# zhangganlin/vista-slam

Hardware: AMD Instinct MI355X
Metric: STA image-pairs/sec @512x384 (higher is better)
Workload: dtype f16x3-split MFMA (3 fp16 products) in the transformer and the pose head; fp16 MFMA + one block-scaled fp8 correction MFMA in the DPT head's convolutions; fp32 accumulate; 1 GPU; 512x384 batch=8 pairs/GPU STA two-view forward (BASELINE configs[1]); pairs_per_gpu=8, H=384, W=512, precision=f16x3h, parallelism=single GPU

## Files before the change

include/sta_mi355_debug.h:

```cpp
#ifndef STA_MI355_DEBUG_H
#define STA_MI355_DEBUG_H
#include "sta_mi355.h"
#ifdef __cplusplus
extern "C" {
#endif

STA_API int sta_set_gemm_variant(sta_handle* h, int variant);

STA_API int sta_debug_pick_family(int amode, int epi, long long M, int N, int K, int split, int cstride, int Ho, int Wo);

STA_API int sta_debug_gemm_plan(int amode, int epi, int M_all, int N, int K, int precision, int mx, int tail_hint, int forced_variant, int* out);

STA_API int sta_debug_last_gemm_plan(sta_handle* h, int* out);

STA_API int sta_debug_qkv_pair_plan(int precision, int M, int N_a, int N_b, int K, int mx_a, int mx_b, int tail_hint, int forced_variant, int* out);

STA_API int sta_debug_qkv_pair(sta_handle* h, const float* x_a, const float* w_a, const float* bias_a, const float* x_b,
                       const float* w_b, const float* bias_b, int S, int ntok, int K, int C, int wp,
                       float* q_a, float* k_a, float* vt_a, float* k_b, float* vt_b, void* stream);

STA_API int sta_debug_gemm(sta_handle* h, const float* A, const float* W, const float* bias, int M, int N, int K,
                   int act, int via_f16, const float* resid, float* out, void* stream);

STA_API int sta_debug_qkv_rope(sta_handle* h, const float* x, const float* W, const float* bias, int S, int ntok, int K, int C,
// ... 14 lines not shown

STA_API int sta_debug_convt(sta_handle* h, const float* x, const float* w, const float* bias, int n, int H, int W, int C, int k,
                    float* out, void* stream);

STA_API int sta_debug_up2(sta_handle* h, const float* x, int n, int H, int W, int C, int Hc, int Wc, float* out, void* stream);

STA_API int sta_debug_layernorm(sta_handle* h, const float* x, const float* g, const float* b, int M, int C, float eps,
                        float* out32, float* out_planes, void* stream);

STA_API int sta_debug_head_final(sta_handle* h, const float* x, const float* w, const float* bias, int64_t npix,
                         float* pts, float* conf, void* stream);

STA_API int sta_debug_svd_orthogonalize(sta_handle* h, const float* m, float* r, int B, void* stream);

STA_API int sta_kernel_timing_dump(sta_handle* h, int cap, double* flops, float* ms, int* variant, int* n_out);

STA_API int sta_kernel_stamps_dump(sta_handle* h, int cap, double* out6, int* n_out);

STA_API int sta_bench_gemm_stamps(sta_handle* h, int M, int N, int K, int resid, double* out, unsigned long long* raw_host, int raw_cap, void* stream);

STA_API int sta_bench_gemm(sta_handle* h, int M, int N, int K, int iters, int tile, int ablation, float* ms_out, void* stream);
STA_API float sta_bench_gemm_last_ghz(void);
STA_API int sta_bench_attention(sta_handle* h, int S, int heads, int nq, int nk, int pose, int iters, int which, float* ms_out, void* stream);

#ifdef __cplusplus
}
#endif
#endif
```

vista_slam_amd/_lib.py:

```python
import ctypes as C
import os

PKG = os.path.dirname(os.path.abspath(__file__))
LIB_PATH = os.path.join(PKG, "libsta_mi355.so")
TEST_LIB_PATH = os.path.join(PKG, "libsta_mi355_test.so")

STA_PREC_F16 = 1
STA_PREC_F16X3 = 3
STA_PREC_F16X3H = 5
STA_PREC_F16X3M = 6
PRECISIONS = {"f16": STA_PREC_F16, "f16x3": STA_PREC_F16X3, "f16x3h": STA_PREC_F16X3H, "f16x3m": STA_PREC_F16X3M}


class StaConfig(C.Structure):
    _fields_ = [("patch_size", C.c_int32), ("enc_embed_dim", C.c_int32), ("enc_depth", C.c_int32),
                ("enc_num_heads", C.c_int32), ("dec_embed_dim", C.c_int32), ("dec_depth", C.c_int32),
                ("dec_num_heads", C.c_int32), ("mlp_ratio", C.c_int32), ("rope_base", C.c_float),
                ("ln_eps", C.c_float), ("precision", C.c_int32)]


_vp, _i, _i64, _f = C.c_void_p, C.c_int, C.c_int64, C.c_float
_fp = C.c_void_p

SIGNATURES = {
# ... 38 lines not shown
    "sta_flops_per_pair": (C.c_double, [_vp, _i, _i]),
    "sta_workspace_bytes": (_i64, [_vp]),
    "sta_weight_bytes": (_i64, [_vp]),
    "sta_enable_stage_timing": (_i, [_vp, _i]),
    "sta_get_stage_ms": (_i, [_vp, C.POINTER(_f)]),
    "sta_kernel_timing": (_i, [_vp, _i]),
    "sta_kernel_timing_read": (_i, [_vp, _i, C.POINTER(_i), C.POINTER(C.c_double), C.POINTER(C.c_double), C.POINTER(C.c_double)]),
    "sta_kernel_clock_read": (_i, [_vp, C.POINTER(C.c_float)]),
    "sta_kernel_timing_filter": (_i, [_vp, _i, _i, _i, _i, _i]),
    "sta_kernel_timing_dump_shapes": (_i, [_vp, _i, C.POINTER(_i), C.POINTER(C.c_float), C.POINTER(_i), C.POINTER(_i)]),
    "sta_range_report": (_i, [_vp, C.POINTER(C.c_ulonglong), _i]),
    "sta_last_error": (C.c_char_p, []),
    "sta_version": (C.c_char_p, []),
}

TEST_SIGNATURES = {
    "sta_set_gemm_variant": (_i, [_vp, _i]),
    "sta_kernel_timing_dump": (_i, [_vp, _i, C.POINTER(C.c_double), C.POINTER(C.c_float), C.POINTER(_i), C.POINTER(_i)]),
    "sta_kernel_stamps_dump": (_i, [_vp, _i, C.POINTER(C.c_double), C.POINTER(_i)]),
    "sta_bench_gemm_stamps": (_i, [_vp, _i, _i, _i, _i, C.POINTER(C.c_double), C.POINTER(C.c_ulonglong), _i, _vp]),
    "sta_bench_gemm": (_i, [_vp, _i, _i, _i, _i, _i, _i, C.POINTER(_f), _vp]),
    "sta_bench_gemm_last_ghz": (C.c_float, []),
    "sta_bench_attention": (_i, [_vp, _i, _i, _i, _i, _i, _i, _i, C.POINTER(_f), _vp]),
    "sta_debug_gemm": (_i, [_vp, _fp, _fp, _fp, _i, _i, _i, _i, _i, _fp, _fp, _vp]),
    "sta_debug_qkv_rope": (_i, [_vp, _fp, _fp, _fp, _i, _i, _i, _i, _i, _i, _fp, _fp, _fp, _vp]),
    "sta_debug_attention": (_i, [_vp, _fp, _fp, _fp, _i, _i, _i, _i, _i, _fp, _vp]),
    "sta_debug_attention_pose": (_i, [_vp, _fp, _fp, _fp, _i, _i, _i, _i, _fp, _vp]),
    "sta_debug_set_tail_hint": (_i, [_vp, _i]),
    "sta_debug_set_option": (_i, [_vp, _i, _i]),
    "sta_debug_pick_family": (_i, [_i, _i, C.c_longlong, _i, _i, _i, _i, _i, _i]),
    "sta_debug_gemm_plan": (_i, [_i, _i, _i, _i, _i, _i, _i, _i, _i, C.POINTER(_i)]),
    "sta_debug_last_gemm_plan": (_i, [_vp, C.POINTER(_i)]),
    "sta_debug_qkv_pair_plan": (_i, [_i, _i, _i, _i, _i, _i, _i, _i, _i, C.POINTER(_i)]),
    "sta_debug_qkv_pair": (_i, [_vp, _fp, _fp, _fp, _fp, _fp, _fp, _i, _i, _i, _i, _i, _fp, _fp, _fp, _fp, _fp, _vp]),
    "sta_debug_conv3x3": (_i, [_vp, _fp, _fp, _fp, _i, _i, _i, _i, _i, _i, _i, _i, _fp, _fp, _vp]),
    "sta_debug_convt": (_i, [_vp, _fp, _fp, _fp, _i, _i, _i, _i, _i, _fp, _vp]),
    "sta_debug_up2": (_i, [_vp, _fp, _i, _i, _i, _i, _i, _i, _fp, _vp]),
    "sta_debug_layernorm": (_i, [_vp, _fp, _fp, _fp, _i, _i, _f, _fp, _fp, _vp]),
    "sta_debug_head_final": (_i, [_vp, _fp, _fp, _fp, _i64, _fp, _fp, _vp]),
    "sta_debug_svd_orthogonalize": (_i, [_vp, _fp, _fp, _i, _vp]),
}

_lib = None
_test_lib = None


# ... 73 lines not shown
```

vista_slam_amd/csrc/attention.h:

```cpp
#pragma once
#include "sta_common.h"
#include <type_traits>

__device__ __forceinline__ void glds16(const void* gsrc, void* lds_dst_wave_base);

struct AttnParams {
    const f16* Q_hi; const f16* Q_lo; const f16* K_hi; const f16* K_lo; const f16* Vt_hi; const f16* Vt_lo;
    f16* O_hi; f16* O_lo; int ldo;
    int S, heads, nq, nk, npad;
    int kv_shift;
    float scale_log2e;
    unsigned long long* range;
    int prefetch;
    int pose;
};

#define ATT_KV 64
#define ATT_TILE_BYTES (64 * 128)

template <bool SPLIT>
constexpr int attn_smem_bytes(int stages = 2) { return stages * (SPLIT ? 4 : 2) * ATT_TILE_BYTES; }
#define ATT_PREFETCH_TILES 4

template <bool SPLIT>
__device__ __forceinline__ void attn_pose_query(const AttnParams& p, char* smem) {
    const int tid = threadIdx.x, lane = tid & 63, wave = tid >> 6;
    const int sh = blockIdx.x;
    const int s = sh / p.heads, h = sh - s * p.heads;
    const int skv = (s + p.kv_shift) % p.S;
    const size_t qoff = ((size_t)(s * p.heads + h) * p.npad + p.nq) * 64;
    const size_t koff = (size_t)(skv * p.heads + h) * p.npad * 64;
    const size_t voff = (size_t)(skv * p.heads + h) * 64 * p.npad;
    float* pl = reinterpret_cast<float*>(smem);
    float* red = pl + p.npad;
    float q[64];
#pragma unroll
    for (int c = 0; c < 8; ++c) {
// ... 42 lines not shown
        H8 a[2], b[2];
#pragma unroll
        for (int u = 0; u < 2; ++u) { a[u].u = ldg16(vh + c0 + u * 8); if (SPLIT) b[u].u = ldg16(vl + c0 + u * 8); }
#pragma unroll
        for (int u = 0; u < 2; ++u) {
            const int c = c0 + u * 8;
            const float4 p0 = *reinterpret_cast<const float4*>(pl + c), p1 = *reinterpret_cast<const float4*>(pl + c + 4);
            const float pe[8] = {p0.x, p0.y, p0.z, p0.w, p1.x, p1.y, p1.z, p1.w};
#pragma unroll
            for (int e = 0; e < 8; ++e) o = __builtin_fmaf(pe[e], (float)a[u].e[e] + (SPLIT ? (float)b[u].e[e] : 0.f), o);
        }
    }
    red[8 + wave * 64 + lane] = o;
    __syncthreads();
    if (wave != 0) return;
    o = (red[8 + lane] + red[8 + 64 + lane]) + (red[8 + 128 + lane] + red[8 + 192 + lane]);
    o /= (red[4] + red[5]) + (red[6] + red[7]);
    const int64_t orow = (int64_t)p.S * p.nq + s, orows = (int64_t)p.S * p.nq + p.S;
    const size_t oo = blk_off<SPLIT>(orow, h * 64 + lane, orows);
    if (SPLIT) { f16 hh, ll; split_f16(o, hh, ll, p.range); p.O_hi[oo] = hh; p.O_hi[oo + 32] = ll; }
    else p.O_hi[oo] = to_f16_sat(o, p.range);
}

template <bool SPLIT>
__global__ __launch_bounds__(256, 2) void attn_kernel(const AttnParams p) {
    extern __shared__ __attribute__((aligned(16))) char smem[];
    constexpr int NPL = SPLIT ? 2 : 1;
    constexpr int STAGE = 2 * NPL * ATT_TILE_BYTES;
    const int npose_blocks = p.pose == 1 ? p.S * p.heads : 0;
    const int nqe = p.nq + (p.pose == 2 ? 1 : 0);
    if ((int)blockIdx.x < npose_blocks) { attn_pose_query<SPLIT>(p, smem); return; }
    const int tid = threadIdx.x, lane = tid & 63;
    const int wave = __builtin_amdgcn_readfirstlane(tid >> 6);
    const int l31 = lane & 31, lhi = lane >> 5;
    const int nqb = (nqe + 127) / 128;
    const int nwg = nqb * p.heads * p.S;
    int logical;
    {
        const int bid = blockIdx.x - npose_blocks, q = nwg / 8, r = nwg % 8, xcd = bid % 8;
        logical = (xcd < r ? xcd * (q + 1) : r * (q + 1) + (xcd - r) * q) + bid / 8;
    }
    const int qb = logical % nqb;
    const int h = (logical / nqb) % p.heads, s = logical / (nqb * p.heads);
    const int skv = (s + p.kv_shift) % p.S;
    const int q0 = qb * 128 + wave * 32;

    const size_t qoff = (size_t)(s * p.heads + h) * p.npad * 64;
    const size_t koff = (size_t)(skv * p.heads + h) * p.npad * 64;
    const size_t voff = (size_t)(skv * p.heads + h) * 64 * p.npad;

    half8 qf_hi[4], qf_lo[4];
    {
        int qrow = q0 + l31; if (qrow > nqe - 1) qrow = nqe - 1;
        const f16* qp = p.Q_hi + qoff + (size_t)qrow * 64 + lhi * 8;
#pragma unroll
        for (int kk = 0; kk < 4; ++kk) { H8 t; t.u = ldg16(qp + kk * 16); qf_hi[kk] = t.h; }
        if (SPLIT) {
            const f16* ql = p.Q_lo + qoff + (size_t)qrow * 64 + lhi * 8;
#pragma unroll
            for (int kk = 0; kk < 4; ++kk) { H8 t; t.u = ldg16(ql + kk * 16); qf_lo[kk] = t.h; }
        }
    }

    int ksrc_l[2], vsrc_l[2];
#pragma unroll
    for (int i = 0; i < 2; ++i) {
        const int row = (2 * wave + i) * 8 + (lane >> 3);
        const int sch = (lane & 7) ^ ((row >> 1) & 7);
        ksrc_l[i] = row * 64 + sch * 8;
        vsrc_l[i] = row * p.npad + sch * 8;
    }
    auto issue_tile = [&](int stage, int kv0) {
        char* sK = smem + stage * STAGE + (2 * wave) * 1024;
        char* sV = sK + NPL * ATT_TILE_BYTES;
#pragma unroll
        for (int i = 0; i < 2; ++i) {
            const size_t ko = koff + (size_t)kv0 * 64 + ksrc_l[i];
            const size_t vo = voff + (size_t)kv0 + vsrc_l[i];
            glds16(p.K_hi + ko, sK + i * 1024);
            glds16(p.Vt_hi + vo, sV + i * 1024);
            if (SPLIT) {
                glds16(p.K_lo + ko, sK + ATT_TILE_BYTES + i * 1024);
                glds16(p.Vt_lo + vo, sV + ATT_TILE_BYTES + i * 1024);
            }
        }
    };

    floatx16 oacc[2];
#pragma unroll
    for (int d = 0; d < 2; ++d)
#pragma unroll
        for (int r = 0; r < 16; ++r) oacc[d][r] = 0.f;
    float m_run = -INFINITY, l_run = 0.f;
    const bool wave_active = q0 < nqe;

    if (p.pose && wave_active) {
        float sp = 0.f;
#pragma unroll
        for (int kk = 0; kk < 4; ++kk) {
            H8 a, b; a.u = ldg16(p.K_hi + koff + (size_t)p.nk * 64 + kk * 16 + lhi * 8);
            if (SPLIT) b.u = ldg16(p.K_lo + koff + (size_t)p.nk * 64 + kk * 16 + lhi * 8);
#pragma unroll
            for (int e = 0; e < 8; ++e) {
                const float kv = (float)a.e[e] + (SPLIT ? (float)b.e[e] : 0.f);
                const float qv = (float)qf_hi[kk][e] + (SPLIT ? (float)qf_lo[kk][e] : 0.f);
                sp = __builtin_fmaf(qv, kv, sp);
            }
        }
        sp += __shfl_xor(sp, 32);
        m_run = sp * p.scale_log2e;
        l_run = lhi == 0 ? 1.f : 0.f;
#pragma unroll
        for (int d = 0; d < 2; ++d)
#pragma unroll
            for (int r = 0; r < 16; ++r) {
                const size_t o = voff + (size_t)(d * 32 + (r & 3) + 8 * (r >> 2) + 4 * lhi) * p.npad + p.nk;
                oacc[d][r] = (float)p.Vt_hi[o] + (SPLIT ? (float)p.Vt_lo[o] : 0.f);
            }
    }

    int foff_l[4];
    {
        const int swz = (l31 >> 1) & 7;
#pragma unroll
        for (int c2 = 0; c2 < 4; ++c2) foff_l[c2] = l31 * 128 + (((c2 * 2 + lhi) ^ swz) << 4);
    }

    auto tile_body = [&](auto stage_c, auto tail_c, int kv0, int stage_rt = 0) {
        constexpr int STG = decltype(stage_c)::value;
        constexpr bool TAIL = decltype(tail_c)::value;
        const char* sK = smem + STG * STAGE + stage_rt * STAGE;
        const char* sV = sK + NPL * ATT_TILE_BYTES;

        floatx16 sacc[2];
#pragma unroll
        for (int t = 0; t < 2; ++t) {
#pragma unroll
            for (int r = 0; r < 16; ++r) sacc[t][r] = 0.f;
#pragma unroll
            for (int kk = 0; kk < 4; ++kk) {
                half8 kf = *reinterpret_cast<const half8*>(sK + t * 4096 + foff_l[kk]);
                if (SPLIT) {
                    half8 kl = *reinterpret_cast<const half8*>(sK + ATT_TILE_BYTES + t * 4096 + foff_l[kk]);
                    sacc[t] = __builtin_amdgcn_mfma_f32_32x32x16_f16(kl, qf_hi[kk], sacc[t], 0, 0, 0);
                    sacc[t] = __builtin_amdgcn_mfma_f32_32x32x16_f16(kf, qf_lo[kk], sacc[t], 0, 0, 0);
                }
                sacc[t] = __builtin_amdgcn_mfma_f32_32x32x16_f16(kf, qf_hi[kk], sacc[t], 0, 0, 0);
            }
        }

        if (TAIL) {
#pragma unroll
            for (int t = 0; t < 2; ++t)
#pragma unroll
                for (int r = 0; r < 16; ++r) {
                    const int key = kv0 + t * 32 + (r & 3) + 8 * (r >> 2) + 4 * lhi;
                    if (key >= p.nk) sacc[t][r] = -INFINITY;
                }
        }
        float mx = -INFINITY;
#pragma unroll
        for (int t = 0; t < 2; ++t)
#pragma unroll
            for (int r = 0; r < 16; ++r) mx = fmaxf(mx, sacc[t][r]);
        mx = fmaxf(mx, __shfl_xor(mx, 32));
        const float m_new = fmaxf(m_run, mx * p.scale_log2e);
        const float alpha = __builtin_amdgcn_exp2f(m_run - m_new);
        const float neg_m = -m_new;
        float psum = 0.f;
#pragma unroll
        for (int t = 0; t < 2; ++t)
#pragma unroll
            for (int r = 0; r < 16; ++r) {
                const float pv = __builtin_amdgcn_exp2f(__builtin_fmaf(sacc[t][r], p.scale_log2e, neg_m));
                sacc[t][r] = pv;
                psum += pv;
            }
        l_run = l_run * alpha + psum;
        m_run = m_new;
        if (!__all(alpha == 1.0f)) {
#pragma unroll
            for (int d = 0; d < 2; ++d)
#pragma unroll
                for (int r = 0; r < 16; ++r) oacc[d][r] *= alpha;
        }

#pragma unroll
        for (int t = 0; t < 2; ++t)
#pragma unroll
            for (int w = 0; w < 2; ++w) {
                union { half8 h; unsigned u[4]; } ph, pl;
#pragma unroll
                for (int j = 0; j < 8; ++j) {
                    const float pv = sacc[t][8 * w + j];
                    const f16 hh = (f16)pv;
                    ph.h[j] = hh;
                    if (SPLIT) pl.h[j] = (f16)(pv - (float)hh);
                }
#pragma unroll
                for (int e = 0; e < 2; ++e) {
                    auto r1 = __builtin_amdgcn_permlane32_swap(ph.u[e], ph.u[2 + e], false, false);
                    ph.u[e] = r1[0]; ph.u[2 + e] = r1[1];
                    if (SPLIT) {
                        auto r2 = __builtin_amdgcn_permlane32_swap(pl.u[e], pl.u[2 + e], false, false);
                        pl.u[e] = r2[0]; pl.u[2 + e] = r2[1];
                    }
                }
                const int c2 = t * 2 + w;
#pragma unroll
                for (int d = 0; d < 2; ++d) {
                    half8 vf = *reinterpret_cast<const half8*>(sV + d * 4096 + foff_l[c2]);
                    if (SPLIT) {
                        half8 vl = *reinterpret_cast<const half8*>(sV + ATT_TILE_BYTES + d * 4096 + foff_l[c2]);
                        oacc[d] = __builtin_amdgcn_mfma_f32_32x32x16_f16(vl, ph.h, oacc[d], 0, 0, 0);
                        oacc[d] = __builtin_amdgcn_mfma_f32_32x32x16_f16(vf, pl.h, oacc[d], 0, 0, 0);
                    }
                    oacc[d] = __builtin_amdgcn_mfma_f32_32x32x16_f16(vf, ph.h, oacc[d], 0, 0, 0);
                }
            }
    };
    using std::integral_constant;
    auto step = [&](auto stage_c, auto tail_c, int it, int ntiles_) {
        constexpr int STG = decltype(stage_c)::value;
        const int kv0 = it * ATT_KV;
        if (it + 1 < ntiles_) issue_tile(STG ^ 1, kv0 + ATT_KV);
        if (wave_active) tile_body(stage_c, tail_c, kv0);
        asm volatile("s_waitcnt vmcnt(0)" ::: "memory");
        __syncthreads();
    };

    const int ntiles = (p.nk + ATT_KV - 1) / ATT_KV, nfull = p.nk / ATT_KV;
    using F = integral_constant<bool, false>; using T = integral_constant<bool, true>;
    if (p.prefetch) {
        constexpr int DMAS = 4 * NPL;
        for (int t = 0; t < ntiles; ++t) issue_tile(t, t * ATT_KV);
        for (int t = 0; t < ntiles; ++t) {
            switch (ntiles - 1 - t) {
                case 3: asm volatile("s_waitcnt vmcnt(%0)" :: "n"(3 * DMAS) : "memory"); break;
                case 2: asm volatile("s_waitcnt vmcnt(%0)" :: "n"(2 * DMAS) : "memory"); break;
                case 1: asm volatile("s_waitcnt vmcnt(%0)" :: "n"(1 * DMAS) : "memory"); break;
                default: asm volatile("s_waitcnt vmcnt(0)" ::: "memory"); break;
            }
            __syncthreads();
            if (wave_active) {
                if (t >= nfull) tile_body(integral_constant<int, 0>{}, T{}, t * ATT_KV, t);
                else tile_body(integral_constant<int, 0>{}, F{}, t * ATT_KV, t);
            }
        }
    } else {
        issue_tile(0, 0);
        asm volatile("s_waitcnt vmcnt(0)" ::: "memory");
        __syncthreads();
        int it = 0;
        for (; it + 1 < nfull; it += 2) {
            step(integral_constant<int, 0>{}, F{}, it, ntiles);
            step(integral_constant<int, 1>{}, F{}, it + 1, ntiles);
        }
        if (it < nfull) { step(integral_constant<int, 0>{}, F{}, it, ntiles); ++it; }
        if (it < ntiles) {
            if (it & 1) step(integral_constant<int, 1>{}, T{}, it, ntiles);
            else step(integral_constant<int, 0>{}, T{}, it, ntiles);
        }
    }

    const float l_tot = l_run + __shfl_xor(l_run, 32);
    const float inv = 1.0f / l_tot;
    const int64_t orows = (int64_t)p.S * p.nq + (p.pose ? p.S : 0);
    if constexpr (SPLIT) {
        __syncthreads();
        char* const wl = smem + wave * (64 * 128);
        RangeAcc ra;
#pragma unroll
        for (int d = 0; d < 2; ++d) {
            const int rowb = (d * 32 + l31) * 128, sw = l31 & 7;
#pragma unroll
            for (int j = 0; j < 2; ++j) {
                union { uint4 u4; unsigned u[4]; } ch, cl;
#pragma unroll
                for (int gg = 0; gg < 2; ++gg) {
                    H4 oh, ol;
#pragma unroll
                    for (int e = 0; e < 4; ++e) split_f16(oacc[d][(2 * j + gg) * 4 + e] * inv, oh.e[e], ol.e[e], ra);
                    ch.u[2 * gg] = oh.u.x; ch.u[2 * gg + 1] = oh.u.y; cl.u[2 * gg] = ol.u.x; cl.u[2 * gg + 1] = ol.u.y;
                }
#pragma unroll
                for (int e = 0; e < 2; ++e) {
                    auto r1 = __builtin_amdgcn_permlane32_swap(ch.u[e], ch.u[2 + e], false, false);
                    ch.u[e] = r1[0]; ch.u[2 + e] = r1[1];
                    auto r2 = __builtin_amdgcn_permlane32_swap(cl.u[e], cl.u[2 + e], false, false);
// ... 39 lines not shown
```

vista_slam_amd/csrc/sta_bench.inc:

```

extern "C" double sta_flops_per_pair(const sta_handle* h, int H, int W) {
    if (!h) return 0;
    const sta_config& c = h->cfg;
    const double E = c.enc_embed_dim, D = c.dec_embed_dim, R = c.mlp_ratio;
    const double hp = H / 16, wp = W / 16, N = hp * wp, Np = N + 1;
    double f_enc = 2 * N * 768 * E + c.enc_depth * ((8 + 4 * R) * N * E * E + 4 * N * N * E);
    double f_dec = 4 * N * E * D + 2.0 * c.dec_depth * ((16 + 4 * R) * Np * D * D + 8 * Np * Np * D);
    auto conv = [](double hh, double ww, double ci, double co, double k) { return 2.0 * hh * ww * ci * co * k * k; };
    double h3 = floor((hp - 1) / 2) + 1, w3 = floor((wp - 1) / 2) + 1;
    double f = 0;
    f += conv(hp, wp, E, 96, 1) + 2.0 * hp * wp * 96 * 96 * 16;
    f += conv(hp, wp, D, 192, 1) + 2.0 * hp * wp * 192 * 192 * 4;
    f += conv(hp, wp, D, 384, 1);
    f += conv(hp, wp, D, 768, 1) + conv(h3, w3, 768, 768, 3);
    f += conv(4 * hp, 4 * wp, 96, 256, 3) + conv(2 * hp, 2 * wp, 192, 256, 3) + conv(hp, wp, 384, 256, 3) + conv(h3, w3, 768, 256, 3);
    f += 2 * conv(h3, w3, 256, 256, 3) + conv(hp, wp, 256, 256, 1);
    f += 4 * conv(hp, wp, 256, 256, 3) + conv(2 * hp, 2 * wp, 256, 256, 1);
    f += 4 * conv(2 * hp, 2 * wp, 256, 256, 3) + conv(4 * hp, 4 * wp, 256, 256, 1);
    f += 4 * conv(4 * hp, 4 * wp, 256, 256, 3) + conv(8 * hp, 8 * wp, 256, 256, 1);
    f += conv(8 * hp, 8 * wp, 256, 128, 3) + conv(16 * hp, 16 * wp, 128, 128, 3) + conv(16 * hp, 16 * wp, 128, 4, 1);
    double f_pose = 2.0 * (D * 512 + 2 * 512 * 512 + 512 * 13);
    return 2 * f_enc + f_dec + 2 * f + 2 * f_pose;
}

// ... 190 lines not shown
    HIPCHK(hipEventSynchronize(e1));
    float ms = 0; HIPCHK(hipEventElapsedTime(&ms, e0, e1));
    std::vector<unsigned long long> hs((size_t)cap * 4);
    HIPCHK(hipMemcpy(hs.data(), stamps, (size_t)cap * 32, hipMemcpyDeviceToHost));
    hipEventDestroy(e0); hipEventDestroy(e1);
    if (raw) memcpy(raw, hs.data(), (size_t)(raw_cap < cap ? raw_cap : cap) * 32);
    std::vector<double> pro, loop, epi, whole;
    unsigned long long t0min = ~0ull, t0max = 0, t3min = ~0ull, t3max = 0;
    for (int b = 0; b < cap; ++b) {
        const unsigned long long* q = &hs[(size_t)b * 4];
        if (!q[3]) continue;
        pro.push_back((double)(q[1] - q[0]) * 0.01); loop.push_back((double)(q[2] - q[1]) * 0.01); epi.push_back((double)(q[3] - q[2]) * 0.01);
        whole.push_back((double)(q[3] - q[0]) * 0.01);
        if (q[0] < t0min) t0min = q[0]; if (q[0] > t0max) t0max = q[0];
        if (q[3] < t3min) t3min = q[3]; if (q[3] > t3max) t3max = q[3];
    }
    REQUIRE(!pro.empty(), "no stamps recorded (this shape did not run on a gemm2 family)");
    auto med = [](std::vector<double>& v) { std::sort(v.begin(), v.end()); return v[v.size() / 2]; };
    out[0] = (double)pro.size(); out[1] = (double)(t3max - t0min) * 0.01; out[2] = med(pro); out[3] = med(loop); out[4] = med(epi);
    out[5] = (double)(t0max - t0min) * 0.01; out[6] = (double)(t3max - t3min) * 0.01; out[7] = ms * 1e3; out[8] = ks; out[9] = med(whole);
    return 0;
}

extern "C" int sta_bench_attention(sta_handle* h, int S, int heads, int nq, int nk, int pose, int iters, int which, float* ms_out, void* stream) {
    REQUIRE(h && ms_out && iters > 0 && S > 0 && heads > 0 && nq > 0 && nk > 0, "bad argument");
    DEV_SCOPE(h->device);
    hipStream_t st = (hipStream_t)stream;
    const bool split = h->prec != STA_PREC_F16;
    const int nmax = (nq > nk ? nq : nk) + (pose ? 1 : 0), npad = rup(nmax, 64);
    const int64_t hsz = (int64_t)S * heads * npad * 64, M = (int64_t)S * nq + (pose ? S : 0);
    CHK(ensure_ws(h, (3 * hsz + M * heads * 64) * 4 + (1 << 16), st));
    h->dry = false;
    Bump ws = cur_bump(h);
    QKVOut o; o.npad = npad; o.q = ws.planes(hsz, true); o.k = ws.planes(hsz, true); o.vt = ws.planes(hsz, true);
    Planes ao = ws.act(M, heads * 64, true);
    REQUIRE(!ws.overflow, "internal: bench workspace overflow");
    if (!split) { o.q.lo = o.k.lo = o.vt.lo = nullptr; ao.lo = nullptr; }
    hipLaunchKernelGGL(fill_rand_f16_kernel, dim3(2048), dim3(256), 0, st, o.q.hi, hsz * 2, 5u, 1.0f);
    hipLaunchKernelGGL(fill_rand_f16_kernel, dim3(2048), dim3(256), 0, st, o.k.hi, hsz * 2, 7u, 1.0f);
    hipLaunchKernelGGL(fill_rand_f16_kernel, dim3(2048), dim3(256), 0, st, o.vt.hi, hsz * 2, 9u, 1.0f);
    REQUIRE(which == 0, "sta_bench_attention: no alternative kernel in this build");
    hipEvent_t e0, e1;
    HIPCHK(hipEventCreate(&e0)); HIPCHK(hipEventCreate(&e1));
    int rc = 0;
    for (int i = 0; i < 2 && rc == 0; ++i) rc = run_attn(h, o, ao, heads * 64, S, heads, nq, nk, 0, st, pose != 0);
    HIPCHK(hipEventRecord(e0, st));
    for (int i = 0; i < iters && rc == 0; ++i) rc = run_attn(h, o, ao, heads * 64, S, heads, nq, nk, 0, st, pose != 0);
    HIPCHK(hipEventRecord(e1, st));
    if (rc != 0) return rc;
    HIPCHK(hipEventSynchronize(e1));
    float ms = 0; HIPCHK(hipEventElapsedTime(&ms, e0, e1));
    *ms_out = ms / iters;
    hipEventDestroy(e0); hipEventDestroy(e1);
    return 0;
}
#endif
```

vista_slam_amd/csrc/sta_launch.inc:

```
template <bool SPLIT, int AMODE, int EPI, int BM, int BN, int WMS, int WNS, int NSTG = 2, bool MX = false>
static int launch_gemm2(const GemmParams& p, hipStream_t st, int dev = 0) {
    static unsigned attr_done = 0;
    constexpr int smem = gemm2_smem_bytes<SPLIT, BM, BN>(NSTG);
    if (!(attr_done >> (dev & 31) & 1u)) {
        HIPCHK(hipFuncSetAttribute((const void*)gemm2_kernel<SPLIT, AMODE, EPI, BM, BN, WMS, WNS, 0, NSTG, MX>,
                                   hipFuncAttributeMaxDynamicSharedMemorySize, smem));
        attr_done |= 1u << (dev & 31);
    }
    int tm = (p.M - p.m_tail + BM - 1) / BM, tn = (p.N + BN - 1) / BN;
    const int ks = p.ksplit > 1 ? p.ksplit : 1;
    const int ntail = p.m_tail > 0 ? (p.N + 31) / 32 : 0;
    hipLaunchKernelGGL((gemm2_kernel<SPLIT, AMODE, EPI, BM, BN, WMS, WNS, 0, NSTG, MX>), dim3((unsigned)(tm * tn * ks + ntail)), dim3(WMS * WNS * 64), smem, st, p);
    return 0;
}

template <bool SPLIT, int EPI, int BM, int BN, bool MX, int WMS = 4, int WNS = 4>
static int launch_conv3h(const GemmParams& p, hipStream_t st, int dev) {
    static unsigned attr_done = 0;
    constexpr int smem = conv3h_smem_bytes<SPLIT, BM, BN>();
    static_assert(smem <= 160 * 1024, "conv3h: LDS budget");
    auto kern = conv3h_kernel<SPLIT, EPI, BM, BN, WMS, WNS, MX>;
    if (!(attr_done >> (dev & 31) & 1u)) {
        HIPCHK(hipFuncSetAttribute((const void*)kern, hipFuncAttributeMaxDynamicSharedMemorySize, smem));
        attr_done |= 1u << (dev & 31);
// ... 537 lines not shown
        if (h->prec != STA_PREC_F16) hipLaunchKernelGGL(resid_ln_kernel<true>, dim3(M), dim3(256), 0, st, p);
        else hipLaunchKernelGGL(resid_ln_kernel<false>, dim3(M), dim3(256), 0, st, p);
        HIPCHK(hipGetLastError());
        return 0;
    }
    dim3 grid((M + 3) / 4);
    if (h->prec != STA_PREC_F16) hipLaunchKernelGGL(ln_kernel<true>, grid, dim3(256), 0, st, p);
    else hipLaunchKernelGGL(ln_kernel<false>, grid, dim3(256), 0, st, p);
    HIPCHK(hipGetLastError());
    return 0;
}

static int rope_fix(sta_handle* h, const Planes& qk, int S, int heads, int npad, int ntok, hipStream_t st) {
    if (h->dry || !h->rope_foreign) return 0;
    const int64_t total = (int64_t)S * heads * (ntok + 1) * 32;
    const dim3 grid((unsigned)((total + 255) / 256));
    if (qk.lo) hipLaunchKernelGGL(rope_planes_kernel<true>, grid, dim3(256), 0, st, qk.hi, qk.lo, S, heads, npad, ntok, h->rope_pos, h->rope_tab, h->range);
    else hipLaunchKernelGGL(rope_planes_kernel<false>, grid, dim3(256), 0, st, qk.hi, qk.lo, S, heads, npad, ntok, h->rope_pos, h->rope_tab, h->range);
    HIPCHK(hipGetLastError());
    return 0;
}

static int run_attn(sta_handle* h, const QKVOut& qkv, const Planes& out, int ldo, int S, int heads,
                    int nq, int nk, int kv_shift, hipStream_t st, bool pose = false) {
    if (h->dry) return 0;
    REQUIRE(!pose || (nq == nk && nq + 1 <= qkv.npad), "internal: pose-token attention needs nq == nk < npad");
    AttnParams p; memset(&p, 0, sizeof p);
    p.range = h->range;
    p.pose = pose ? (nq % 128 != 0 ? 2 : 1) : 0;
    p.Q_hi = qkv.q.hi; p.Q_lo = qkv.q.lo; p.K_hi = qkv.k.hi; p.K_lo = qkv.k.lo; p.Vt_hi = qkv.vt.hi; p.Vt_lo = qkv.vt.lo;
    p.O_hi = out.hi; p.O_lo = out.lo; p.ldo = ldo;
    p.S = S; p.heads = heads; p.nq = nq; p.nk = nk; p.npad = qkv.npad; p.kv_shift = kv_shift;
    p.scale_log2e = 0.125f * 1.44269504088896340736f;
    const int npose = p.pose == 1 ? S * heads : 0;
    REQUIRE(!pose || (int64_t)(qkv.npad + 8 + 256) * 4 <= attn_smem_bytes<false>(), "internal: pose-query scratch exceeds the LDS allocation");
    REQUIRE(!pose || qkv.npad % 64 == 0, "internal: pose-query path needs npad % 64 == 0");
    dim3 grid((unsigned)(((nq + (p.pose == 2 ? 1 : 0) + 127) / 128) * heads * S + npose));
    p.prefetch = (nk <= ATT_PREFETCH_TILES * ATT_KV && grid.x <= 256 && h->opt[5] != 1) ? 1 : 0;
    const int stages = p.prefetch ? ATT_PREFETCH_TILES : 2;
    if (h->prec != STA_PREC_F16) {
        static unsigned attr_done = 0;
        if (!(attr_done >> (h->device & 31) & 1u)) { hipFuncSetAttribute((const void*)attn_kernel<true>, hipFuncAttributeMaxDynamicSharedMemorySize, attn_smem_bytes<true>(ATT_PREFETCH_TILES)); attr_done |= 1u << (h->device & 31); }
        hipLaunchKernelGGL(attn_kernel<true>, grid, dim3(256), attn_smem_bytes<true>(stages), st, p);
    } else {
        STA_F16ONLY(hipLaunchKernelGGL(attn_kernel<false>, grid, dim3(256), attn_smem_bytes<false>(stages), st, p));
    }
    HIPCHK(hipGetLastError());
    return 0;
}

static int run_rows_to_planes(sta_handle* h, const float* x, int64_t bstride, int nb, int rows, int C, const Planes& o, hipStream_t st, int64_t obstride = 0, bool mx = false) {
// ... 45 lines not shown
```

Before: 196.5 pairs/s.

## Switch attention MFMAs from 32x32x16 to 16x16x32 with two query sub-blocks

Rewrites the flash-attention inner loop to use 16x16x32 f16 MFMAs with each wave holding two 16-row query blocks, and changes the K LDS swizzle and fragment offsets to match. Row max and sum reductions move to permlane16/32 swaps, and the accumulators are repacked into the old 32x32 layout before the epilogue. K and V fragments are read from LDS ahead of the MFMA chains, with sched barriers placed to overlap LDS reads with compute. It also adds an optional per-block clock-stamp path and a clock benchmark entry point, which cost a pointer check in the kernel when unused.

```diff
diff --git a/include/sta_mi355_debug.h b/include/sta_mi355_debug.h
--- a/include/sta_mi355_debug.h
+++ b/include/sta_mi355_debug.h
@@ -60,6 +60,7 @@
 STA_API int sta_bench_gemm(sta_handle* h, int M, int N, int K, int iters, int tile, int ablation, float* ms_out, void* stream);
 STA_API float sta_bench_gemm_last_ghz(void);
 STA_API int sta_bench_attention(sta_handle* h, int S, int heads, int nq, int nk, int pose, int iters, int which, float* ms_out, void* stream);
+STA_API int sta_bench_attention_clock(sta_handle* h, int S, int heads, int nq, int nk, int pose, double warm_s, double* out, void* stream);
 
 #ifdef __cplusplus
 }
diff --git a/vista_slam_amd/_lib.py b/vista_slam_amd/_lib.py
--- a/vista_slam_amd/_lib.py
+++ b/vista_slam_amd/_lib.py
@@ -84,6 +84,7 @@
     "sta_bench_gemm": (_i, [_vp, _i, _i, _i, _i, _i, _i, C.POINTER(_f), _vp]),
     "sta_bench_gemm_last_ghz": (C.c_float, []),
     "sta_bench_attention": (_i, [_vp, _i, _i, _i, _i, _i, _i, _i, C.POINTER(_f), _vp]),
+    "sta_bench_attention_clock": (_i, [_vp, _i, _i, _i, _i, _i, C.c_double, C.POINTER(C.c_double), _vp]),
     "sta_debug_gemm": (_i, [_vp, _fp, _fp, _fp, _i, _i, _i, _i, _i, _fp, _fp, _vp]),
     "sta_debug_qkv_rope": (_i, [_vp, _fp, _fp, _fp, _i, _i, _i, _i, _i, _i, _fp, _fp, _fp, _vp]),
     "sta_debug_attention": (_i, [_vp, _fp, _fp, _fp, _i, _i, _i, _i, _i, _fp, _vp]),
diff --git a/vista_slam_amd/csrc/attention.h b/vista_slam_amd/csrc/attention.h
--- a/vista_slam_amd/csrc/attention.h
+++ b/vista_slam_amd/csrc/attention.h
@@ -13,6 +13,7 @@
     unsigned long long* range;
     int prefetch;
     int pose;
+    unsigned long long* stamps;
 };
 
 #define ATT_KV 64
@@ -101,6 +102,21 @@
     else p.O_hi[oo] = to_f16_sat(o, p.range);
 }
 
+__device__ __forceinline__ float lanegroup_sum(float x) {
+    const auto a = __builtin_amdgcn_permlane16_swap(__float_as_uint(x), __float_as_uint(x), false, false);
+    x = __uint_as_float(a[0]) + __uint_as_float(a[1]);
+    const auto b = __builtin_amdgcn_permlane32_swap(__float_as_uint(x), __float_as_uint(x), false, false);
+    return __uint_as_float(b[0]) + __uint_as_float(b[1]);
+}
+__device__ __forceinline__ void lanegroup_max2(float& x0, float& x1) {
+    const auto a = __builtin_amdgcn_permlane16_swap(__float_as_uint(x0), __float_as_uint(x1), false, false);
+    float y = fmaxf(__uint_as_float(a[0]), __uint_as_float(a[1]));
+    const auto b = __builtin_amdgcn_permlane32_swap(__float_as_uint(y), __float_as_uint(y), false, false);
+    y = fmaxf(__uint_as_float(b[0]), __uint_as_float(b[1]));
+    const auto c = __builtin_amdgcn_permlane16_swap(__float_as_uint(y), __float_as_uint(y), false, false);
+    x0 = __uint_as_float(c[0]); x1 = __uint_as_float(c[1]);
+}
+
 template <bool SPLIT>
 __global__ __launch_bounds__(256, 2) void attn_kernel(const AttnParams p) {
     extern __shared__ __attribute__((aligned(16))) char smem[];
@@ -109,6 +125,8 @@
     const int npose_blocks = p.pose == 1 ? p.S * p.heads : 0;
     const int nqe = p.nq + (p.pose == 2 ? 1 : 0);
     if ((int)blockIdx.x < npose_blocks) { attn_pose_query<SPLIT>(p, smem); return; }
+    unsigned long long clk0 = 0, rt0 = 0;
+    if (p.stamps) { clk0 = __builtin_amdgcn_s_memtime(); rt0 = __builtin_amdgcn_s_memrealtime(); }
     const int tid = threadIdx.x, lane = tid & 63;
     const int wave = __builtin_amdgcn_readfirstlane(tid >> 6);
     const int l31 = lane & 31, lhi = lane >> 5;
@@ -128,16 +146,16 @@
     const size_t koff = (size_t)(skv * p.heads + h) * p.npad * 64;
     const size_t voff = (size_t)(skv * p.heads + h) * 64 * p.npad;
 
-    half8 qf_hi[4], qf_lo[4];
-    {
-        int qrow = q0 + l31; if (qrow > nqe - 1) qrow = nqe - 1;
-        const f16* qp = p.Q_hi + qoff + (size_t)qrow * 64 + lhi * 8;
-#pragma unroll
-        for (int kk = 0; kk < 4; ++kk) { H8 t; t.u = ldg16(qp + kk * 16); qf_hi[kk] = t.h; }
-        if (SPLIT) {
-            const f16* ql = p.Q_lo + qoff + (size_t)qrow * 64 + lhi * 8;
-#pragma unroll
-            for (int kk = 0; kk < 4; ++kk) { H8 t; t.u = ldg16(ql + kk * 16); qf_lo[kk] = t.h; }
+    const int l15 = lane & 15, lg = lane >> 4;
+    half8 qf_hi[2][2], qf_lo[2][2];
+#pragma unroll
+    for (int qb = 0; qb < 2; ++qb) {
+        int qrow = q0 + 16 * qb + l15; if (qrow > nqe - 1) qrow = nqe - 1;
+        const size_t qo = qoff + (size_t)qrow * 64 + lg * 8;
+#pragma unroll
+        for (int ks = 0; ks < 2; ++ks) {
+            H8 t; t.u = ldg16(p.Q_hi + qo + ks * 32); qf_hi[qb][ks] = t.h;
+            if (SPLIT) { t.u = ldg16(p.Q_lo + qo + ks * 32); qf_lo[qb][ks] = t.h; }
         }
     }
 
@@ -145,9 +163,8 @@
 #pragma unroll
     for (int i = 0; i < 2; ++i) {
         const int row = (2 * wave + i) * 8 + (lane >> 3);
-        const int sch = (lane & 7) ^ ((row >> 1) & 7);
-        ksrc_l[i] = row * 64 + sch * 8;
-        vsrc_l[i] = row * p.npad + sch * 8;
+        ksrc_l[i] = row * 64 + (((lane & 7) ^ (((row >> 1) & 1) | ((row >> 2) & 6))) * 8);
+        vsrc_l[i] = row * p.npad + (((lane & 7) ^ ((row >> 1) & 7)) * 8);
     }
     auto issue_tile = [&](int stage, int kv0) {
         char* sK = smem + stage * STAGE + (2 * wave) * 1024;
@@ -165,44 +182,52 @@
         }
     };
 
-    floatx16 oacc[2];
-#pragma unroll
-    for (int d = 0; d < 2; ++d)
-#pragma unroll
-        for (int r = 0; r < 16; ++r) oacc[d][r] = 0.f;
-    float m_run = -INFINITY, l_run = 0.f;
+    floatx4 oacc4[4][2];
+#pragma unroll
+    for (int db = 0; db < 4; ++db)
+#pragma unroll
+        for (int qb = 0; qb < 2; ++qb) oacc4[db][qb] = floatx4{0.f, 0.f, 0.f, 0.f};
+    float m_run[2] = {-INFINITY, -INFINITY}, l_run[2] = {0.f, 0.f};
     const bool wave_active = q0 < nqe;
 
     if (p.pose && wave_active) {
-        float sp = 0.f;
-#pragma unroll
-        for (int kk = 0; kk < 4; ++kk) {
-            H8 a, b; a.u = ldg16(p.K_hi + koff + (size_t)p.nk * 64 + kk * 16 + lhi * 8);
-            if (SPLIT) b.u = ldg16(p.K_lo + koff + (size_t)p.nk * 64 + kk * 16 + lhi * 8);
+        float sp[2] = {0.f, 0.f};
+#pragma unroll
+        for (int ks = 0; ks < 2; ++ks) {
+            H8 a, b; a.u = ldg16(p.K_hi + koff + (size_t)p.nk * 64 + ks * 32 + lg * 8);
+            if (SPLIT) b.u = ldg16(p.K_lo + koff + (size_t)p.nk * 64 + ks * 32 + lg * 8);
 #pragma unroll
             for (int e = 0; e < 8; ++e) {
                 const float kv = (float)a.e[e] + (SPLIT ? (float)b.e[e] : 0.f);
-                const float qv = (float)qf_hi[kk][e] + (SPLIT ? (float)qf_lo[kk][e] : 0.f);
-                sp = __builtin_fmaf(qv, kv, sp);
-            }
-        }
-        sp += __shfl_xor(sp, 32);
-        m_run = sp * p.scale_log2e;
-        l_run = lhi == 0 ? 1.f : 0.f;
-#pragma unroll
-        for (int d = 0; d < 2; ++d)
-#pragma unroll
-            for (int r = 0; r < 16; ++r) {
-                const size_t o = voff + (size_t)(d * 32 + (r & 3) + 8 * (r >> 2) + 4 * lhi) * p.npad + p.nk;
-                oacc[d][r] = (float)p.Vt_hi[o] + (SPLIT ? (float)p.Vt_lo[o] : 0.f);
-            }
-    }
-
-    int foff_l[4];
+#pragma unroll
+                for (int qb = 0; qb < 2; ++qb)
+                    sp[qb] = __builtin_fmaf((float)qf_hi[qb][ks][e] + (SPLIT ? (float)qf_lo[qb][ks][e] : 0.f), kv, sp[qb]);
+            }
+        }
+#pragma unroll
+        for (int qb = 0; qb < 2; ++qb) {
+            m_run[qb] = lanegroup_sum(sp[qb]) * p.scale_log2e;
+            l_run[qb] = lg == 0 ? 1.f : 0.f;
+        }
+#pragma unroll
+        for (int db = 0; db < 4; ++db)
+#pragma unroll
+            for (int i = 0; i < 4; ++i) {
+                const size_t o = voff + (size_t)(16 * db + 8 * (lg & 1) + 4 * (lg >> 1) + i) * p.npad + p.nk;
+                const float v = (float)p.Vt_hi[o] + (SPLIT ? (float)p.Vt_lo[o] : 0.f);
+                oacc4[db][0][i] = v; oacc4[db][1][i] = v;
+            }
+    }
+
+    int koff_l[2], voff_l[2];
     {
-        const int swz = (l31 >> 1) & 7;
-#pragma unroll
-        for (int c2 = 0; c2 < 4; ++c2) foff_l[c2] = l31 * 128 + (((c2 * 2 + lhi) ^ swz) << 4);
+        const int krow = 8 * (l15 >> 2) + (l15 & 3), kswz = ((krow >> 1) & 1) | ((krow >> 2) & 6);
+        const int vrow = 8 * ((l15 >> 2) & 1) + 4 * (l15 >> 3) + (l15 & 3), vswz = (vrow >> 1) & 7;
+#pragma unroll
+        for (int j = 0; j < 2; ++j) {
+            koff_l[j] = krow * 128 + (((4 * j + lg) ^ kswz) << 4);
+            voff_l[j] = vrow * 128 + (((4 * j + lg) ^ vswz) << 4);
+        }
     }
 
     auto tile_body = [&](auto stage_c, auto tail_c, int kv0, int stage_rt = 0) {
@@ -211,92 +236,115 @@
         const char* sK = smem + STG * STAGE + stage_rt * STAGE;
         const char* sV = sK + NPL * ATT_TILE_BYTES;
 
-        floatx16 sacc[2];
-#pragma unroll
-        for (int t = 0; t < 2; ++t) {
-#pragma unroll
-            for (int r = 0; r < 16; ++r) sacc[t][r] = 0.f;
-#pragma unroll
-            for (int kk = 0; kk < 4; ++kk) {
-                half8 kf = *reinterpret_cast<const half8*>(sK + t * 4096 + foff_l[kk]);
+        half8 kf[4][2], kl[4][2];
+#pragma unroll
+        for (int kb = 0; kb < 4; ++kb)
+#pragma unroll
+            for (int ks = 0; ks < 2; ++ks) {
+                const int o = (kb >> 1) * 4096 + (kb & 1) * 512 + koff_l[ks];
+                kf[kb][ks] = *reinterpret_cast<const half8*>(sK + o);
+                if (SPLIT) kl[kb][ks] = *reinterpret_cast<const half8*>(sK + ATT_TILE_BYTES + o);
+            }
+        __builtin_amdgcn_sched_barrier(0);
+        floatx4 sacc[4][2];
+#pragma unroll
+        for (int kb = 0; kb < 4; ++kb) {
+#pragma unroll
+            for (int qb = 0; qb < 2; ++qb) sacc[kb][qb] = floatx4{0.f, 0.f, 0.f, 0.f};
+#pragma unroll
+            for (int ks = 0; ks < 2; ++ks) {
                 if (SPLIT) {
-                    half8 kl = *reinterpret_cast<const half8*>(sK + ATT_TILE_BYTES + t * 4096 + foff_l[kk]);
-                    sacc[t] = __builtin_amdgcn_mfma_f32_32x32x16_f16(kl, qf_hi[kk], sacc[t], 0, 0, 0);
-                    sacc[t] = __builtin_amdgcn_mfma_f32_32x32x16_f16(kf, qf_lo[kk], sacc[t], 0, 0, 0);
-                }
-                sacc[t] = __builtin_amdgcn_mfma_f32_32x32x16_f16(kf, qf_hi[kk], sacc[t], 0, 0, 0);
-            }
-        }
+#pragma unroll
+                    for (int qb = 0; qb < 2; ++qb) {
+                        sacc[kb][qb] = __builtin_amdgcn_mfma_f32_16x16x32_f16(kl[kb][ks], qf_hi[qb][ks], sacc[kb][qb], 0, 0, 0);
+                        sacc[kb][qb] = __builtin_amdgcn_mfma_f32_16x16x32_f16(kf[kb][ks], qf_lo[qb][ks], sacc[kb][qb], 0, 0, 0);
+                    }
+                }
+#pragma unroll
+                for (int qb = 0; qb < 2; ++qb) sacc[kb][qb] = __builtin_amdgcn_mfma_f32_16x16x32_f16(kf[kb][ks], qf_hi[qb][ks], sacc[kb][qb], 0, 0, 0);
+            }
+        }
+        half8 vf[2][4], vl[2][4];
+        auto read_v = [&](int c) {
+#pragma unroll
+            for (int db = 0; db < 4; ++db) {
+                vf[c][db] = *reinterpret_cast<const half8*>(sV + db * 2048 + voff_l[c]);
+                if (SPLIT) vl[c][db] = *reinterpret_cast<const half8*>(sV + ATT_TILE_BYTES + db * 2048 + voff_l[c]);
+            }
+        };
+        read_v(0);
+        __builtin_amdgcn_sched_barrier(0);
 
         if (TAIL) {
 #pragma unroll
-            for (int t = 0; t < 2; ++t)
-#pragma unroll
-                for (int r = 0; r < 16; ++r) {
-                    const int key = kv0 + t * 32 + (r & 3) + 8 * (r >> 2) + 4 * lhi;
-                    if (key >= p.nk) sacc[t][r] = -INFINITY;
-                }
-        }
-        float mx = -INFINITY;
-#pragma unroll
-        for (int t = 0; t < 2; ++t)
-#pragma unroll
-            for (int r = 0; r < 16; ++r) mx = fmaxf(mx, sacc[t][r]);
-        mx = fmaxf(mx, __shfl_xor(mx, 32));
-        const float m_new = fmaxf(m_run, mx * p.scale_log2e);
-        const float alpha = __builtin_amdgcn_exp2f(m_run - m_new);
-        const float neg_m = -m_new;
-        float psum = 0.f;
-#pragma unroll
-        for (int t = 0; t < 2; ++t)
-#pragma unroll
-            for (int r = 0; r < 16; ++r) {
-                const float pv = __builtin_amdgcn_exp2f(__builtin_fmaf(sacc[t][r], p.scale_log2e, neg_m));
-                sacc[t][r] = pv;
-                psum += pv;
-            }
-        l_run = l_run * alpha + psum;
-        m_run = m_new;
-        if (!__all(alpha == 1.0f)) {
-#pragma unroll
-            for (int d = 0; d < 2; ++d)
-#pragma unroll
-                for (int r = 0; r < 16; ++r) oacc[d][r] *= alpha;
-        }
-
-#pragma unroll
-        for (int t = 0; t < 2; ++t)
-#pragma unroll
-            for (int w = 0; w < 2; ++w) {
-                union { half8 h; unsigned u[4]; } ph, pl;
+            for (int kb = 0; kb < 4; ++kb)
+#pragma unroll
+                for (int i = 0; i < 4; ++i) {
+                    const int key = kv0 + 32 * (kb >> 1) + 8 * lg + 4 * (kb & 1) + i;
+                    if (key >= p.nk) { sacc[kb][0][i] = -INFINITY; sacc[kb][1][i] = -INFINITY; }
+                }
+        }
+        float mx[2] = {-INFINITY, -INFINITY};
+#pragma unroll
+        for (int qb = 0; qb < 2; ++qb)
+#pragma unroll
+            for (int kb = 0; kb < 4; ++kb)
+#pragma unroll
+                for (int i = 0; i < 4; ++i) mx[qb] = fmaxf(mx[qb], sacc[kb][qb][i]);
+        lanegroup_max2(mx[0], mx[1]);
+        float alpha[2], neg_m[2], psum[2] = {0.f, 0.f};
+#pragma unroll
+        for (int qb = 0; qb < 2; ++qb) {
+            const float m_new = fmaxf(m_run[qb], mx[qb] * p.scale_log2e);
+            alpha[qb] = __builtin_amdgcn_exp2f(m_run[qb] - m_new);
+            neg_m[qb] = -m_new;
+            m_run[qb] = m_new;
+        }
+#pragma unroll
+        for (int kb = 0; kb < 4; ++kb)
+#pragma unroll
+            for (int qb = 0; qb < 2; ++qb)
+#pragma unroll
+                for (int i = 0; i < 4; ++i) {
+                    const float pv = __builtin_amdgcn_exp2f(__builtin_fmaf(sacc[kb][qb][i], p.scale_log2e, neg_m[qb]));
+                    sacc[kb][qb][i] = pv;
+                    psum[qb] += pv;
+                }
+#pragma unroll
+        for (int qb = 0; qb < 2; ++qb) l_run[qb] = l_run[qb] * alpha[qb] + psum[qb];
+        if (!__all(alpha[0] == 1.0f && alpha[1] == 1.0f)) {
+#pragma unroll
+            for (int db = 0; db < 4; ++db)
+#pragma unroll
+                for (int qb = 0; qb < 2; ++qb) oacc4[db][qb] *= alpha[qb];
+        }
+
+#pragma unroll
+        for (int c = 0; c < 2; ++c) {
+            half8 ph[2], pl[2];
+            if (c == 0) read_v(1);
+#pragma unroll
+            for (int qb = 0; qb < 2; ++qb)
 #pragma unroll
                 for (int j = 0; j < 8; ++j) {
-                    const float pv = sacc[t][8 * w + j];
+                    const float pv = sacc[2 * c + (j >> 2)][qb][j & 3];
                     const f16 hh = (f16)pv;
-                    ph.h[j] = hh;
-                    if (SPLIT) pl.h[j] = (f16)(pv - (float)hh);
-                }
-#pragma unroll
-                for (int e = 0; e < 2; ++e) {
-                    auto r1 = __builtin_amdgcn_permlane32_swap(ph.u[e], ph.u[2 + e], false, false);
-                    ph.u[e] = r1[0]; ph.u[2 + e] = r1[1];
-                    if (SPLIT) {
-                        auto r2 = __builtin_amdgcn_permlane32_swap(pl.u[e], pl.u[2 + e], false, false);
-                        pl.u[e] = r2[0]; pl.u[2 + e] = r2[1];
+                    ph[qb][j] = hh;
+                    if (SPLIT) pl[qb][j] = (f16)(pv - (float)hh);
+                }
+#pragma unroll
+            for (int db = 0; db < 4; ++db) {
+                if (SPLIT) {
+#pragma unroll
+                    for (int qb = 0; qb < 2; ++qb) {
+                        oacc4[db][qb] = __builtin_amdgcn_mfma_f32_16x16x32_f16(vl[c][db], ph[qb], oacc4[db][qb], 0, 0, 0);
+                        oacc4[db][qb] = __builtin_amdgcn_mfma_f32_16x16x32_f16(vf[c][db], pl[qb], oacc4[db][qb], 0, 0, 0);
                     }
                 }
-                const int c2 = t * 2 + w;
-#pragma unroll
-                for (int d = 0; d < 2; ++d) {
-                    half8 vf = *reinterpret_cast<const half8*>(sV + d * 4096 + foff_l[c2]);
-                    if (SPLIT) {
-                        half8 vl = *reinterpret_cast<const half8*>(sV + ATT_TILE_BYTES + d * 4096 + foff_l[c2]);
-                        oacc[d] = __builtin_amdgcn_mfma_f32_32x32x16_f16(vl, ph.h, oacc[d], 0, 0, 0);
-                        oacc[d] = __builtin_amdgcn_mfma_f32_32x32x16_f16(vf, pl.h, oacc[d], 0, 0, 0);
-                    }
-                    oacc[d] = __builtin_amdgcn_mfma_f32_32x32x16_f16(vf, ph.h, oacc[d], 0, 0, 0);
-                }
-            }
+#pragma unroll
+                for (int qb = 0; qb < 2; ++qb) oacc4[db][qb] = __builtin_amdgcn_mfma_f32_16x16x32_f16(vf[c][db], ph[qb], oacc4[db][qb], 0, 0, 0);
+            }
+        }
     };
     using std::integral_constant;
     auto step = [&](auto stage_c, auto tail_c, int it, int ntiles_) {
@@ -342,8 +390,23 @@
         }
     }
 
-    const float l_tot = l_run + __shfl_xor(l_run, 32);
-    const float inv = 1.0f / l_tot;
+    floatx16 oacc[2];
+#pragma unroll
+    for (int db = 0; db < 4; ++db)
+#pragma unroll
+        for (int i = 0; i < 4; ++i) {
+            const auto xy = __builtin_amdgcn_permlane16_swap(__float_as_uint(oacc4[db][0][i]), __float_as_uint(oacc4[db][1][i]), false, false);
+            oacc[db >> 1][8 * (db & 1) + i] = __uint_as_float(xy[0]);
+            oacc[db >> 1][8 * (db & 1) + 4 + i] = __uint_as_float(xy[1]);
+        }
+    if (p.stamps && threadIdx.x == 0) {
+        asm volatile("" ::"v"(oacc[0][0]), "v"(oacc[1][15]) : "memory");
+        unsigned long long* o = p.stamps + (size_t)(blockIdx.x - npose_blocks) * 4;
+        o[0] = clk0; o[1] = rt0; o[2] = __builtin_amdgcn_s_memtime(); o[3] = __builtin_amdgcn_s_memrealtime();
+    }
+
+    const float l_q0 = lanegroup_sum(l_run[0]), l_q1 = lanegroup_sum(l_run[1]);
+    const float inv = 1.0f / ((lg & 1) ? l_q1 : l_q0);
     const int64_t orows = (int64_t)p.S * p.nq + (p.pose ? p.S : 0);
     if constexpr (SPLIT) {
         __syncthreads();
diff --git a/vista_slam_amd/csrc/sta_bench.inc b/vista_slam_amd/csrc/sta_bench.inc
--- a/vista_slam_amd/csrc/sta_bench.inc
+++ b/vista_slam_amd/csrc/sta_bench.inc
@@ -236,23 +236,32 @@
     return 0;
 }
 
-extern "C" int sta_bench_attention(sta_handle* h, int S, int heads, int nq, int nk, int pose, int iters, int which, float* ms_out, void* stream) {
-    REQUIRE(h && ms_out && iters > 0 && S > 0 && heads > 0 && nq > 0 && nk > 0, "bad argument");
-    DEV_SCOPE(h->device);
-    hipStream_t st = (hipStream_t)stream;
+static int attn_bench_operands(sta_handle* h, int S, int heads, int nq, int nk, int pose, hipStream_t st, QKVOut& o, Planes& ao,
+                               unsigned long long** stamps = nullptr, int64_t stamp_cap = 0) {
     const bool split = h->prec != STA_PREC_F16;
     const int nmax = (nq > nk ? nq : nk) + (pose ? 1 : 0), npad = rup(nmax, 64);
     const int64_t hsz = (int64_t)S * heads * npad * 64, M = (int64_t)S * nq + (pose ? S : 0);
-    CHK(ensure_ws(h, (3 * hsz + M * heads * 64) * 4 + (1 << 16), st));
+    CHK(ensure_ws(h, (3 * hsz + M * heads * 64) * 4 + stamp_cap * 32 + (1 << 16), st));
     h->dry = false;
     Bump ws = cur_bump(h);
-    QKVOut o; o.npad = npad; o.q = ws.planes(hsz, true); o.k = ws.planes(hsz, true); o.vt = ws.planes(hsz, true);
-    Planes ao = ws.act(M, heads * 64, true);
+    o.npad = npad; o.q = ws.planes(hsz, true); o.k = ws.planes(hsz, true); o.vt = ws.planes(hsz, true);
+    ao = ws.act(M, heads * 64, true);
+    if (stamps) *stamps = (unsigned long long*)ws.take(stamp_cap * 32);
     REQUIRE(!ws.overflow, "internal: bench workspace overflow");
     if (!split) { o.q.lo = o.k.lo = o.vt.lo = nullptr; ao.lo = nullptr; }
     hipLaunchKernelGGL(fill_rand_f16_kernel, dim3(2048), dim3(256), 0, st, o.q.hi, hsz * 2, 5u, 1.0f);
     hipLaunchKernelGGL(fill_rand_f16_kernel, dim3(2048), dim3(256), 0, st, o.k.hi, hsz * 2, 7u, 1.0f);
     hipLaunchKernelGGL(fill_rand_f16_kernel, dim3(2048), dim3(256), 0, st, o.vt.hi, hsz * 2, 9u, 1.0f);
+    HIPCHK(hipGetLastError());
+    return 0;
+}
+
+extern "C" int sta_bench_attention(sta_handle* h, int S, int heads, int nq, int nk, int pose, int iters, int which, float* ms_out, void* stream) {
+    REQUIRE(h && ms_out && iters > 0 && S > 0 && heads > 0 && nq > 0 && nk > 0, "bad argument");
+    DEV_SCOPE(h->device);
+    hipStream_t st = (hipStream_t)stream;
+    QKVOut o; Planes ao;
+    CHK(attn_bench_operands(h, S, heads, nq, nk, pose, st, o, ao));
     REQUIRE(which == 0, "sta_bench_attention: no alternative kernel in this build");
     hipEvent_t e0, e1;
     HIPCHK(hipEventCreate(&e0)); HIPCHK(hipEventCreate(&e1));
@@ -268,4 +277,48 @@
     hipEventDestroy(e0); hipEventDestroy(e1);
     return 0;
 }
-#endif
+
+extern "C" int sta_bench_attention_clock(sta_handle* h, int S, int heads, int nq, int nk, int pose, double warm_s, double* out, void* stream) {
+    REQUIRE(h && out && S > 0 && heads > 0 && nq > 0 && nk > 0 && warm_s >= 0, "bad argument");
+    DEV_SCOPE(h->device);
+    hipStream_t st = (hipStream_t)stream;
+    const int64_t cap = (int64_t)((nq + 1 + 127) / 128) * heads * S;
+    QKVOut o; Planes ao; unsigned long long* stamps = nullptr;
+    CHK(attn_bench_operands(h, S, heads, nq, nk, pose, st, o, ao, &stamps, cap));
+    hipEvent_t e0, e1;
+    HIPCHK(hipEventCreate(&e0)); HIPCHK(hipEventCreate(&e1));
+    int rc = 0;
+    float ms = 0;
+    for (int i = 0; i < 2 && rc == 0; ++i) rc = run_attn(h, o, ao, heads * 64, S, heads, nq, nk, 0, st, pose != 0);
+    HIPCHK(hipEventRecord(e0, st));
+    for (int i = 0; i < 20 && rc == 0; ++i) rc = run_attn(h, o, ao, heads * 64, S, heads, nq, nk, 0, st, pose != 0);
+    HIPCHK(hipEventRecord(e1, st));
+    if (rc != 0) return rc;
+    HIPCHK(hipEventSynchronize(e1));
+    HIPCHK(hipEventElapsedTime(&ms, e0, e1));
+    const int iters = (int)std::min(2000000.0, std::ceil(warm_s * 1e3 / std::max(ms / 20, 1e-3f)));
+    HIPCHK(hipEventRecord(e0, st));
+    for (int i = 0; i < iters && rc == 0; ++i) rc = run_attn(h, o, ao, heads * 64, S, heads, nq, nk, 0, st, pose != 0);
+    HIPCHK(hipEventRecord(e1, st));
+    HIPCHK(hipMemsetAsync(stamps, 0, (size_t)cap * 32, st));
+    if (rc == 0) rc = run_attn(h, o, ao, heads * 64, S, heads, nq, nk, 0, st, pose != 0, stamps);
+    if (rc != 0) return rc;
+    HIPCHK(hipStreamSynchronize(st));
+    HIPCHK(hipEventElapsedTime(&ms, e0, e1));
+    hipEventDestroy(e0); hipEventDestroy(e1);
+    std::vector<unsigned long long> hs((size_t)cap * 4);
+    HIPCHK(hipMemcpy(hs.data(), stamps, (size_t)cap * 32, hipMemcpyDeviceToHost));
+    std::vector<double> ghz, us;
+    for (int64_t b = 0; b < cap; ++b) {
+        const unsigned long long* q = &hs[(size_t)b * 4];
+        if (!q[3] || q[3] <= q[1]) continue;
+        ghz.push_back((double)(q[2] - q[0]) / (double)(q[3] - q[1]) * 0.1);
+        us.push_back((double)(q[3] - q[1]) * 0.01);
+    }
+    REQUIRE(!ghz.empty(), "no stamps recorded");
+    std::sort(ghz.begin(), ghz.end()); std::sort(us.begin(), us.end());
+    out[0] = ghz[ghz.size() / 2]; out[1] = ghz.front(); out[2] = ghz.back(); out[3] = (double)ghz.size();
+    out[4] = (double)ms * 1e3 / (iters > 0 ? iters : 1); out[5] = us[us.size() / 2];
+    return 0;
+}
+#endif
diff --git a/vista_slam_amd/csrc/sta_launch.inc b/vista_slam_amd/csrc/sta_launch.inc
--- a/vista_slam_amd/csrc/sta_launch.inc
+++ b/vista_slam_amd/csrc/sta_launch.inc
@@ -583,11 +583,12 @@
 }
 
 static int run_attn(sta_handle* h, const QKVOut& qkv, const Planes& out, int ldo, int S, int heads,
-                    int nq, int nk, int kv_shift, hipStream_t st, bool pose = false) {
+                    int nq, int nk, int kv_shift, hipStream_t st, bool pose = false, unsigned long long* stamps = nullptr) {
     if (h->dry) return 0;
     REQUIRE(!pose || (nq == nk && nq + 1 <= qkv.npad), "internal: pose-token attention needs nq == nk < npad");
     AttnParams p; memset(&p, 0, sizeof p);
     p.range = h->range;
+    p.stamps = stamps;
     p.pose = pose ? (nq % 128 != 0 ? 2 : 1) : 0;
     p.Q_hi = qkv.q.hi; p.Q_lo = qkv.q.lo; p.K_hi = qkv.k.hi; p.K_lo = qkv.k.lo; p.Vt_hi = qkv.vt.hi; p.Vt_lo = qkv.vt.lo;
     p.O_hi = out.hi; p.O_lo = out.lo; p.ldo = ldo;
```

Measured after the change: 197.8 pairs/s, median of 6. Within noise of the previous version (+0.6%).
